# zertovitch/zip-ada

Hardware: AMD Instinct MI355X
Metric: Deflate encode MB/s (Deflate_3; stream bit-exact with the CPU restatement of the reference, Ada parity unpinned) (higher is better)
Workload: dtype u8

## Files before the change

### zip-ada_amd/csrc/zada_logic.h

```cpp
#pragma once
#include <type_traits>
#include <stdint.h>

#if defined(__HIPCC__)
#define ZADA_HD __host__ __device__ __forceinline__
#else
#define ZADA_HD inline
#endif

namespace zada {

constexpr uint32_t TOK_MATCH = 0x80000000u;
ZADA_HD uint32_t tok_match(uint32_t len, uint32_t dist) { return TOK_MATCH | (len << 16) | dist; }
ZADA_HD bool tok_is_match(uint32_t t) { return (t & TOK_MATCH) != 0; }
ZADA_HD uint32_t tok_len(uint32_t t) { return tok_is_match(t) ? ((t >> 16) & 0x1FF) : 1u; }
ZADA_HD uint32_t tok_dist(uint32_t t) { return t & 0xFFFF; }

constexpr int MIN_MATCH = 3, MAX_MATCH = 258, MAX_DIST = 32506, TOO_FAR = 4096;
constexpr int WSIZE = 32768;

struct LzConfig { int good, lazy, nice, chain; };
ZADA_HD LzConfig lz_config(int level) {
  switch (level) {
    case 4: return {4, 4, 16, 16};
// ... 71 lines not shown
}


struct MatchPair { uint32_t full, quarter; };
constexpr uint32_t M_GUESS = 0x80000000u, M_DEMAND = 0x40000000u, M_BYSPEC = 0x20000000u, M_HAVEQ = 0x10000000u, M_VALUE = 0x01FFFFFFu;
constexpr uint32_t M_BEAT_SHIFT = 25, M_BEAT_MAX = 127;
struct NoGuess { ZADA_HD void operator()(uint32_t, uint32_t, uint32_t, uint32_t) const {} };
struct ParseIO { const uint8_t *in; uint64_t n; const MatchPair *M; LzConfig cfg; const uint32_t *segend; };
struct Layout { const uint32_t *segend; uint64_t n; };
struct ExitState { uint32_t pos, kind; };

struct BitmapWriter {
  uint32_t *bits; uint64_t word; uint32_t acc;
  ZADA_HD void init(uint32_t *b, uint64_t first) { bits = b; acc = 0; word = first; }
  ZADA_HD void set(uint64_t p) {
    uint64_t w = p >> 5;
    while (word < w) { bits[word] = acc; acc = 0; word++; }
    acc |= 1u << (p & 31);
  }
  ZADA_HD void finish(uint64_t last) {
    while (word < last) { bits[word] = acc; acc = 0; word++; }
    bits[word] = acc;
  }
};

struct DirectFetch { const MatchPair *M; ZADA_HD MatchPair operator()(uint32_t p) const { return M[p]; } };
template <typename F> struct has_byte { template <typename U> static auto test(int) -> decltype(((U *)0)->byte(0u), char()); template <typename U> static long test(...); static const bool value = sizeof(test<F>(0)) == 1; };
template <typename F> ZADA_HD typename std::enable_if<has_byte<typename std::remove_reference<F>::type>::value, uint32_t>::type fetch_byte(F &f, const uint8_t *, uint32_t p) { return f.byte(p); }
template <typename F> ZADA_HD typename std::enable_if<!has_byte<typename std::remove_reference<F>::type>::value, uint32_t>::type fetch_byte(F &, const uint8_t *in, uint32_t p) { return in[p]; }
struct DirectSink { uint32_t *tok; uint32_t &ntok; ZADA_HD void push(uint32_t t) { tok[ntok++] = t; } };
struct CappedSink { uint32_t *tok; uint32_t &ntok; uint32_t cap; uint32_t *overflow; ZADA_HD void push(uint32_t t) { if (ntok < cap) tok[ntok] = t; else if (overflow) *overflow = 1u; ntok++; } };
template <typename Sink, typename OnTop, typename OnGuess, typename Fetch>
ZADA_HD void run_parser(ParseState &s, const ParseIO &io, Sink &&sink, OnTop &&on_top, OnGuess &&on_guess, Fetch &&fetch) {
  for (;;) {
    if ((uint64_t)s.p >= io.n) {
      if (s.avail) { sink.push(io.in[io.n - 1]); s.avail = 0; s.mlen = 2; }
      return;
    }
    if (on_top(s)) return;
    const uint64_t la = io.n - s.p;
    const bool srch = parse_searches(s, io.cfg, la);
    uint32_t m = 0;
    if (srch) {
      const MatchPair mm = fetch(s.p);
      if (mm.full & M_GUESS) on_guess(s.p, mm.full, mm.quarter, s.mlen);
      m = (parse_need_quarter(s, io.cfg) ? mm.quarter : mm.full) & M_VALUE;
    }
    const uint32_t bb = s.avail ? fetch_byte(fetch, io.in, s.p - 1) : 0;
    const uint32_t t = parse_step(s, m, srch, bb);
    if (t != 0xFFFFFFFFu) sink.push(t);
  }
}

template <typename Sink, typename OnGuess, typename Fetch>
ZADA_HD void parse_spec_chunk_to(const ParseIO &io, uint32_t k, uint32_t chunk, Sink &&sink,
                                 uint32_t *Fbits, uint32_t *Lbits, ExitState &ex, OnGuess on_guess, Fetch &&fetch) {
  const uint64_t c0 = (uint64_t)k * chunk, c1 = (c0 + chunk < io.n) ? c0 + chunk : io.n;
  ParseState s{(uint32_t)c0, 0, 2, 0};
  BitmapWriter fw, lw;
  fw.init(Fbits, c0 >> 5); lw.init(Lbits, c0 >> 5);
  ExitState e; e.pos = (uint32_t)io.n; e.kind = SYNC_F;
  run_parser(s, io, sink, [&](const ParseState &st) {
    int kind = sync_kind(st);
    if (kind == SYNC_NONE) return false;
    if ((uint64_t)st.p >= c1) { e.pos = st.p; e.kind = (uint32_t)kind; return true; }
    if (kind == SYNC_F) fw.set(st.p); else lw.set(st.p);
    return false;
  }, on_guess, fetch);
  const uint64_t lastw = c1 > c0 ? (c1 - 1) >> 5 : c0 >> 5;
  fw.finish(lastw);
  lw.finish(lastw);
  ex = e;
}
template <typename OnGuess, typename Fetch>
ZADA_HD void parse_spec_chunk(const ParseIO &io, uint32_t k, uint32_t chunk, uint32_t *tok, uint32_t &ntok,
                              uint32_t *Fbits, uint32_t *Lbits, ExitState &ex, OnGuess on_guess, Fetch &&fetch) {
  parse_spec_chunk_to(io, k, chunk, DirectSink{tok, ntok}, Fbits, Lbits, ex, on_guess, fetch);
}
ZADA_HD void parse_spec_chunk(const ParseIO &io, uint32_t k, uint32_t chunk, uint32_t *tok, uint32_t &ntok,
                              uint32_t *Fbits, uint32_t *Lbits, ExitState &ex) {
  parse_spec_chunk_to(io, k, chunk, DirectSink{tok, ntok}, Fbits, Lbits, ex, NoGuess(), DirectFetch{io.M});
}

template <typename OnGuess, typename Fetch>
ZADA_HD void parse_fix_chunk(const ParseIO &io, uint32_t k, uint32_t chunk, ExitState entry,
                             const uint32_t *spec_tok, uint32_t spec_cnt, const uint32_t *Fbits, const uint32_t *Lbits,
                             ExitState spec_exit, uint32_t *tok, uint32_t &ntok, uint32_t &take, uint32_t &u0, ExitState &new_exit,
                             OnGuess on_guess, Fetch &&fetch, uint32_t tok_cap = 0xFFFFFFFFu, uint32_t *tok_overflow = nullptr) {
  const uint64_t c0 = (uint64_t)k * chunk, c1 = (c0 + chunk < io.n) ? c0 + chunk : io.n;
  u0 = entry.kind == SYNC_L ? entry.pos - 1 : entry.pos;
  ntok = 0;
  if ((uint64_t)entry.pos >= c1) {
    new_exit = entry; take = spec_cnt;
    return;
  }
  ParseState s{entry.pos, entry.kind == SYNC_L ? 1u : 0u, 2, 0};
  bool synced = false;
  ExitState e; e.pos = (uint32_t)io.n; e.kind = SYNC_F;
  run_parser(s, io, CappedSink{tok, ntok, tok_cap, tok_overflow}, [&](const ParseState &st) {
    int kind = sync_kind(st);
    if (kind == SYNC_NONE) return false;
    if ((uint64_t)st.p >= c1) { e.pos = st.p; e.kind = (uint32_t)kind; return true; }
    uint32_t wbits = (kind == SYNC_F ? Fbits : Lbits)[st.p >> 5];
    if ((wbits >> (st.p & 31)) & 1) { synced = true; e.pos = st.p; e.kind = (uint32_t)kind; return true; }
    return false;
  }, on_guess, fetch);
  if (synced) {
    const uint32_t u = e.kind == SYNC_L ? e.pos - 1 : e.pos;
    uint32_t cur = (uint32_t)c0, j = 0;
    while (cur < u) { cur += tok_len(spec_tok[j]); j++; }
    take = j;
    new_exit = spec_exit;
  } else {
    take = spec_cnt;
    new_exit = e;
  }
}
ZADA_HD void parse_fix_chunk(const ParseIO &io, uint32_t k, uint32_t chunk, ExitState entry,
                                    const uint32_t *spec_tok, uint32_t spec_cnt, const uint32_t *Fbits, const uint32_t *Lbits,
                                    ExitState spec_exit, uint32_t *tok, uint32_t &ntok, uint32_t &take, uint32_t &u0, ExitState &new_exit) {
  parse_fix_chunk(io, k, chunk, entry, spec_tok, spec_cnt, Fbits, Lbits, spec_exit, tok, ntok, take, u0, new_exit, NoGuess(), DirectFetch{io.M});
}

template <typename T>
ZADA_HD void patch_dist_stats(T *sd) {
  int used = 0;
  for (int i = 0; i < 32; i++) if (sd[i] != 0) used++;
  if (used == 0) { sd[0] = 1; sd[1] = 1; }
  else if (used == 1) { if (sd[0] == 0) sd[0] = 1; else sd[1] = 1; }
}

ZADA_HD void tweak_for_better_rle(uint32_t *counts, int counts_len, uint8_t *good) {
  int length = counts_len, stride;
  uint32_t symbol, sum, limit, new_count;
  for (int i = 0; i < counts_len; i++) good[i] = 0;
  for (;;) { if (length == 0) return; if (counts[length - 1] != 0) break; length--; }
  symbol = counts[0]; stride = 0;
  for (int i = 0; i <= length; i++) {
    if (i == length || counts[i] != symbol) {
      if ((symbol == 0 && stride >= 5) || (symbol != 0 && stride >= 7))
        for (int k = 0; k < stride; k++) good[i - k - 1] = 1;
      stride = 1;
      if (i != length) symbol = counts[i];
    } else stride++;
  }
  stride = 0; limit = counts[0]; sum = 0;
  for (int i = 0; i <= length; i++) {
    bool brk = (i == length) || good[i] || (i > 0 && good[i - 1]);
    if (!brk) { int64_t d = (int64_t)counts[i] - (int64_t)limit; if (d < 0) d = -d; brk = d >= 4; }
    if (brk) {
      if (stride >= 4 || (stride >= 3 && sum == 0)) {
        new_count = (sum + (uint32_t)stride / 2) / (uint32_t)stride;
        if (new_count < 1) new_count = 1;
        if (sum == 0) new_count = 0;
        for (int k = 0; k < stride; k++) counts[i - k - 1] = new_count;
      }
      stride = 0; sum = 0;
      if (i < length - 3) limit = (counts[i] + counts[i + 1] + counts[i + 2] + counts[i + 3] + 2) / 4;
      else if (i < length) limit = counts[i];
      else limit = 0;
    }
    stride++;
    if (i != length) sum += counts[i];
  }
}

// ... 62 lines not shown
```

### zip-ada_amd/csrc/zada_lz.hip

```cpp
#include <hip/hip_runtime.h>
#include <mutex>
#include <stdint.h>
#include "zada_logic.h"
#include "zada_internal.h"
#include <chrono>
#include <stdio.h>
#include <stdlib.h>
#include <vector>

namespace zada {

typedef uint32_t __attribute__((aligned(1))) u32u;
typedef uint64_t __attribute__((aligned(1))) u64u;
#define RL(v, j) ((uint32_t)__builtin_amdgcn_readlane((int)(v), (j)))
#define RL64(v, j) ((uint64_t)RL((uint32_t)(v), (j)) | ((uint64_t)RL((uint32_t)((v) >> 32), (j)) << 32))

#ifndef ZADA_NO_XCD_MAP
__device__ __forceinline__ uint32_t xcd_block() {
  const uint32_t n = gridDim.x, full = n & ~7u, b = blockIdx.x;
  return b < full ? (b & 7u) * (full >> 3) + (b >> 3) : b;
}
#else
__device__ __forceinline__ uint32_t xcd_block() { return blockIdx.x; }
#endif
// ... 1373 lines not shown
      };
      uint32_t s_end = lds_u32(WI + (uint32_t)bst - 3);
      bool over = false;
      auto batch = [&](uint32_t d) {
        const bool valid = d != 0;
        const bool inr = valid && d <= LF;
        bool pass = false;
        if (inr) pass = lds_u32(WI - d + (uint32_t)bst - 3) == s_end;
        unsigned long long pm = __ballot(pass);
        while (pm) {
          const int j = __ffsll((long long)pm) - 1;
          const uint32_t dj = RL(d, j);
          if (!hq && dj > LQ) { hq = true; rqq = bst >= 3 ? ((uint32_t)bst << 16) | bd : 0u; }
          const uint32_t o = 4u * (uint32_t)lane;
          const uint32_t x = lds_u32(WI - dj + o) ^ lds_u32(WI + o);
          const unsigned long long mm = __ballot(x != 0);
          int len;
          if (mm) { const int l0 = __ffsll((long long)mm) - 1; len = 4 * l0 + (int)(__builtin_ctz(RL(x, l0)) >> 3); }
          else { const uint32_t y = LDS_U16(win8, WI - dj + 256) ^ LDS_U16(win8, WI + 256); len = 256 + (y == 0 ? 2 : ((y & 0xFF) == 0 ? 1 : 0)); }
          len = len < LA ? len : LA;
          if (len > bst) {
            bst = len; bd = dj;
            if (len >= NICE) { over = true; break; }
            s_end = lds_u32(WI + (uint32_t)bst - 3);
            pass = pass && lane > j && lds_u32(WI - d + (uint32_t)bst - 3) == s_end;
          } else pass = pass && lane > j;
          pm = __ballot(pass);
        }
        if (!over && !hq && __any(valid && d > LQ)) { hq = true; rqq = bst >= 3 ? ((uint32_t)bst << 16) | bd : 0u; }
        if (__any(!inr)) over = true;
      };
      uint32_t dq[DM_AHEAD];
      dq[0] = r0;
#pragma unroll
      for (int u = 1; u < DM_AHEAD; u++) dq[u] = 64u * u < TT ? cand_load(ds, 64u * u + (uint32_t)lane) : 0u;
      for (uint32_t c0 = 0; c0 < TT && !over; c0 += 64 * DM_AHEAD) {
#pragma unroll
        for (int u = 0; u < DM_AHEAD; u++) {
          if (c0 + 64u * u < TT && !over) {
            const uint32_t dcur = cand_dist(ds, c0 + 64u * u + (uint32_t)lane, dq[u]);
            const uint32_t cn = c0 + 64u * (u + DM_AHEAD);
            if (cn < TT) dq[u] = cand_load(ds, cn + (uint32_t)lane);
            batch(dcur);
          }
        }
      }
      if (lane == 0) {
        const uint32_t packed = bst >= 3 ? ((uint32_t)bst << 16) | bd : 0u;
        store_result(B + ds.k, packed, hq ? rqq : packed, ds.og_full, ds.og_quarter, (ds.best_hq >> 14) & 1u);
      }
    }
    __syncthreads();
    DM_STAMP(3);
  }
}

__global__ void k_demand_all(Layout L, MatchPair *__restrict__ M, uint32_t *__restrict__ blk_demand, uint32_t *__restrict__ dbits) {
  const uint64_t p = (uint64_t)blockIdx.x * blockDim.x + threadIdx.x;
  if (p >= L.n || p >= lay_end(L, p >> 15)) return;
  const uint32_t f = M[p].full;
  if (f & M_GUESS) {
    if (!(f & M_DEMAND)) M[p].full = f | M_DEMAND | M_BYSPEC;
    atomicOr(&dbits[p >> 5], 1u << (p & 31));
    blk_demand[p / DMB] = 1;
  }
}

struct DemandMarker {
  MatchPair *M; uint32_t *blk_demand; uint32_t *n_demand; uint32_t by;
  bool track = false;
  uint32_t *dbits;
  __device__ void operator()(uint32_t p, uint32_t full, uint32_t quarter, uint32_t beat) const {
    if (track && (beat < M_BEAT_MAX ? beat : M_BEAT_MAX) < (quarter >> M_BEAT_SHIFT))
      __hip_atomic_fetch_min(&M[p].quarter, (quarter & M_VALUE) | ((beat < M_BEAT_MAX ? beat : M_BEAT_MAX) << M_BEAT_SHIFT), __ATOMIC_RELAXED, __HIP_MEMORY_SCOPE_AGENT);
    const uint32_t want = M_DEMAND | by;
    if ((full & want) == want) return;
    M[p].full = full | want;
    atomicOr(&dbits[p >> 5], 1u << (p & 31));
    blk_demand[p / DMB] = 1;
    *n_demand = 1;
  }
};

#ifndef ZADA_PS_BWORDS
#define ZADA_PS_BWORDS 16
#endif
#ifndef ZADA_PS_TOKS
#define ZADA_PS_TOKS 8
#endif
constexpr uint32_t PS_BWORDS = ZADA_PS_BWORDS, PS_TOKS = ZADA_PS_TOKS;
static_assert((PS_BWORDS == 8 || PS_BWORDS == 16) && (PS_TOKS == 4 || PS_TOKS == 8), "line sizes of the parser's LDS caches");
struct LineFetch {
  const MatchPair *M; uint64_t *slot;
  uint32_t tag;
  __device__ MatchPair operator()(uint32_t p) {
    const uint32_t t = p >> 3;
    if (t != tag) {
      const uint4 *src = (const uint4 *)(M + ((uint64_t)t << 3));
      const uint4 a = src[0], b = src[1], c = src[2], d = src[3];
      slot[0 * 64] = (uint64_t)a.x | ((uint64_t)a.y << 32); slot[1 * 64] = (uint64_t)a.z | ((uint64_t)a.w << 32);
      slot[2 * 64] = (uint64_t)b.x | ((uint64_t)b.y << 32); slot[3 * 64] = (uint64_t)b.z | ((uint64_t)b.w << 32);
      slot[4 * 64] = (uint64_t)c.x | ((uint64_t)c.y << 32); slot[5 * 64] = (uint64_t)c.z | ((uint64_t)c.w << 32);
      slot[6 * 64] = (uint64_t)d.x | ((uint64_t)d.y << 32); slot[7 * 64] = (uint64_t)d.z | ((uint64_t)d.w << 32);
      tag = t;
    }
    const uint64_t v = slot[(p & 7u) * 64];
    MatchPair r; r.full = (uint32_t)v; r.quarter = (uint32_t)(v >> 32);
    return r;
  }
  const uint8_t *in; uint32_t *bslot; uint32_t btag;
  __device__ uint32_t byte(uint32_t p) {
    constexpr uint32_t SH = PS_BWORDS == 16 ? 6 : 5;
    const uint32_t t = p >> SH;
    if (t != btag) {
      const uint4 *src = (const uint4 *)(in + ((uint64_t)t << SH));
      const uint4 a = src[0], b = src[1];
      bslot[0 * 64] = a.x; bslot[1 * 64] = a.y; bslot[2 * 64] = a.z; bslot[3 * 64] = a.w;
      bslot[4 * 64] = b.x; bslot[5 * 64] = b.y; bslot[6 * 64] = b.z; bslot[7 * 64] = b.w;
      if (PS_BWORDS == 16) {
        const uint4 c = src[2], d = src[3];
        bslot[8 * 64] = c.x; bslot[9 * 64] = c.y; bslot[10 * 64] = c.z; bslot[11 * 64] = c.w;
        bslot[12 * 64] = d.x; bslot[13 * 64] = d.y; bslot[14 * 64] = d.z; bslot[15 * 64] = d.w;
      }
      btag = t;
    }
    return (bslot[((p >> 2) & (PS_BWORDS - 1u)) * 64] >> (8 * (p & 3u))) & 0xFFu;
  }
};

struct TokSink {
  uint32_t *dst; uint32_t *buf; uint32_t n;
  __device__ void push(uint32_t t) {
    buf[(n & (PS_TOKS - 1u)) * 64] = t;
    n++;
    if ((n & (PS_TOKS - 1u)) == 0) {
      uint4 a;
      a.x = buf[0]; a.y = buf[64]; a.z = buf[128]; a.w = buf[192];
      uint4 *o = (uint4 *)(dst + n - PS_TOKS);
      o[0] = a;
      if (PS_TOKS == 8) { uint4 b; b.x = buf[256]; b.y = buf[320]; b.z = buf[384]; b.w = buf[448]; o[1] = b; }
    }
  }
  __device__ void flush() { for (uint32_t i = n & ~(PS_TOKS - 1u); i < n; i++) dst[i] = buf[(i & (PS_TOKS - 1u)) * 64]; }
};

__global__ void __launch_bounds__(1024) k_list_flagged(const uint8_t *__restrict__ flag, uint32_t n, uint32_t *__restrict__ list, uint32_t *__restrict__ count) {
  __shared__ uint32_t wcnt[16], wbase;
  const uint32_t i = blockIdx.x * 1024 + threadIdx.x, lane = threadIdx.x & 63, w = threadIdx.x >> 6;
  const bool f = i < n && flag[i];
  const unsigned long long mk = __ballot(f);
  if (lane == 0) wcnt[w] = (uint32_t)__popcll(mk);
  __syncthreads();
  if (threadIdx.x == 0) {
    uint32_t t = 0;
    for (int k = 0; k < 16; k++) { const uint32_t c = wcnt[k]; wcnt[k] = t; t += c; }
    wbase = t ? atomicAdd(count, t) : 0u;
  }
  __syncthreads();
  if (f) list[wbase + wcnt[w] + (uint32_t)__popcll(mk & ((1ull << lane) - 1ull))] = i;
}

#ifdef ZADA_RESPEC_STATS
__device__ unsigned long long g_respec_dbg[4];
#endif
__global__ void k_parse_spec(ParseIO io, uint32_t nchunks, uint32_t *__restrict__ spec_tok, uint32_t *__restrict__ spec_cnt,
                             uint32_t *__restrict__ Fbits, uint32_t *__restrict__ Lbits, ExitState *__restrict__ exits,
                             DemandMarker dm, const uint32_t *__restrict__ list , const uint32_t *__restrict__ list_n,
                             uint32_t exact_max ) {
  uint32_t k = blockIdx.x * blockDim.x + threadIdx.x;
  if (list) {
    const uint32_t nl = *list_n;
    if (nl <= exact_max || k >= nl) return;
    k = list[k];
  }
  if (k >= nchunks) return;
  if (io.segend) io.n = io.segend[((uint64_t)k * PCHUNK) >> 15] & 0x7FFFFFFFu;
  uint32_t ntok = 0;
  ExitState ex;
#ifdef ZADA_RESPEC_STATS
  uint32_t old_h = 0, old_n = 0; ExitState old_ex{0, 0};
  if (list) { old_n = spec_cnt[k]; old_ex = exits[k]; const uint32_t *ot = spec_tok + (uint64_t)k * PTOK_STRIDE; for (uint32_t i = 0; i < old_n; i++) old_h = old_h * 0x9E3779B1u + ot[i]; }
#endif
  __shared__ uint64_t lines[8 * 64];
  __shared__ uint32_t tbuf[PS_TOKS * 64];
  __shared__ uint32_t blines[PS_BWORDS * 64];
  LineFetch lf; lf.M = io.M; lf.slot = lines + threadIdx.x; lf.tag = 0xFFFFFFFFu; lf.in = io.in; lf.bslot = blines + threadIdx.x; lf.btag = 0xFFFFFFFFu;
  TokSink ts; ts.dst = spec_tok + (uint64_t)k * PTOK_STRIDE; ts.buf = tbuf + threadIdx.x; ts.n = 0;
  parse_spec_chunk_to(io, k, PCHUNK, ts, Fbits, Lbits, ex, dm, lf);
  ts.flush();
  ntok = ts.n;
  spec_cnt[k] = ntok;
  exits[k] = ex;
#ifdef ZADA_RESPEC_STATS
  if (list) {
    __threadfence();
    uint32_t new_h = 0; const uint32_t *nt = spec_tok + (uint64_t)k * PTOK_STRIDE; for (uint32_t i = 0; i < ntok; i++) new_h = new_h * 0x9E3779B1u + nt[i];
    atomicAdd(&g_respec_dbg[0], 1ull);
    if (new_h == old_h && ntok == old_n && ex.pos == old_ex.pos && ex.kind == old_ex.kind) atomicAdd(&g_respec_dbg[1], 1ull);
  }
#endif
}

struct WaveExact {
  const uint8_t *in; Layout L; DistPlanes dp; RunPtrs rp; const uint16_t *tailsK; MatchPair *M; int nice_cfg; const uint16_t *resume;
  __device__ __forceinline__ uint32_t g32(uint64_t o) const { return *(const u32u *)(in + o); }
  __device__ MatchPair search(uint64_t p, MatchPair og) const {
    const int lane = threadIdx.x & 63;
    const uint64_t seg = p >> 15, n = lay_end(L, seg);
    const bool seg_first = lay_first(L, seg), prev_first = seg > 0 && lay_first(L, seg - 1);
    const uint64_t rem = n - p;
    const int la = rem < 258 ? (int)rem : 258;
    const int nice = nice_cfg < la ? nice_cfg : la;
    const uint64_t pbase = (seg << 15) - 32768;
    const uint32_t dlimv = dp.limits(p);
    uint32_t dl[NLEVELS];
#pragma unroll
    for (int l = 0; l < NLEVELS; l++) dl[l] = dp.d[l][p];
    const uint32_t idx1 = rp.idx[p], c1 = rp.cnt[p];
    uint32_t t = 0xFFFFu;
    if (!seg_first) {
      const uint32_t key = hashL_of(*(const u64u *)(in + p), 3 + NLEVELS);
      const uint32_t tt = tailsK[(seg - 1) * 65536ull + key];
      const uint64_t q = pbase + tt;
      if (tt < lay_inserted(L, seg - 1) && p - q <= (uint64_t)MAX_DIST && hashL_of(*(const u64u *)(in + q), 3 + NLEVELS) == key) t = tt;
    }
    uint32_t idx2 = 0, c2 = 0;
    if (t != 0xFFFFu) { idx2 = rp.idx[pbase + t]; c2 = (uint32_t)rp.cnt[pbase + t] + 1u; }
    const uint32_t df = dlimv & 0xFFFF, dq = dlimv >> 16;
    const uint32_t LF = dl[0] == (uint32_t)MAX_DIST ? (uint32_t)MAX_DIST : (df < (uint32_t)(MAX_DIST - 1) ? df : (uint32_t)(MAX_DIST - 1));
    const uint32_t LQ = dq < LF ? dq : LF;
    int bst = 2;
    uint32_t bd = 0, rqq = 0;
    bool chain_ok = true;
#pragma unroll
    for (int l = 0; l < NLEVELS; l++) {
      const bool v = la >= 3 + l && dl[l] != 0 && dl[l] <= LF;
      if (v) { bst = 3 + l; bd = dl[l]; if (dl[l] <= LQ) rqq = ((uint32_t)(3 + l) << 16) | dl[l]; }
      chain_ok = v;
    }
    bool hq = chain_ok && bd > LQ;
    uint32_t i1 = idx1, n1 = c1, i2 = idx2, n2 = c2;
    if (chain_ok) {
      const uint32_t gl = (og.full & M_VALUE) >> 16;
      if (gl >= 3) { bst = (int)gl; bd = og.full & 0xFFFFu; }
      hq = (og.full & M_HAVEQ) != 0;
      if (hq) rqq = og.quarter & M_VALUE;
      const uint64_t q = p - resume[p];
      const uint32_t iq = rp.idx[q];
      const uint32_t skip = q >= (seg << 15) ? idx1 - 1 - iq : c1 + (idx2 - iq);
      if (skip < c1) { i1 = idx1 - skip; n1 = c1 - skip; }
      else { const uint32_t s2 = skip - c1 < c2 ? skip - c1 : c2; n1 = 0; i2 = idx2 - s2; n2 = c2 - s2; }
    }
    MatchPair r;
    if (!(chain_ok && bst < nice && n1 + n2 > 0)) {
      const uint32_t packed = bst >= 3 ? ((uint32_t)bst << 16) | bd : 0u;
      r.full = packed; r.quarter = !chain_ok ? rqq : (hq ? rqq : packed);
      if (lane == 0) M[p] = r;
      return r;
    }
    const uint16_t *sprev = rp.S + ((seg << 15) - 32768);
    const uint32_t TT = n1 + n2, po = (uint32_t)p & 32767u;
    auto cand = [&](uint32_t c) -> uint32_t {
      const bool in1 = c < n1, in2 = !in1 && c - n1 < n2;
      const uint32_t a = in1 ? 32768u + i1 - 1u - c : (in2 ? i2 - (c - n1) : 32768u);
      const uint32_t raw = sprev[a];
      const bool q0 = raw == 0 && ((in1 && seg_first) || (in2 && prev_first));
      return q0 ? 0u : (in1 ? po - raw : (in2 ? po + 32768u - raw : 0u));
    };
    uint32_t s_end = g32(p + (uint32_t)bst - 3);
    bool over = false;
    uint32_t dnext = cand((uint32_t)lane);
    for (uint32_t c0 = 0; c0 < TT && !over; c0 += 64) {
      const uint32_t d = dnext;
      if (c0 + 64 < TT) dnext = cand(c0 + 64 + (uint32_t)lane);
      const bool valid = d != 0;
      const bool inr = valid && d <= LF;
      bool pass = false;
      if (inr) pass = g32(p - d + (uint32_t)bst - 3) == s_end;
      unsigned long long pm = __ballot(pass);
      while (pm) {
        const int j = __ffsll((long long)pm) - 1;
        const uint32_t dj = RL(d, j);
// ... 341 lines not shown
        const uint32_t s1 = s0 + PIECE < nseg ? s0 + PIECE : nseg;
        const uint64_t upto = (uint64_t)s1 * 32768 + 64 < n ? (uint64_t)s1 * 32768 + 64 : n;
        if (int rn = job.need(upto)) return rn;
        const auto t_now = std::chrono::steady_clock::now();
        const bool slow = s0 > 0 && std::chrono::duration<double>(t_now - t_prev).count() >= SLOW_PIECE_S;
        t_prev = t_now;
        prev_links(s0, s1);
#ifndef ZADA_OLD_INIT
        if (s0 == 0) hipStreamWaitEvent(st, c->ev_dlim, 0);
#endif
        if (slow) cross_links_upto(s1);
        hipLaunchKernelGGL(k_bucket_limits, dim3(s1 - s0), dim3(256), 0, st, L, cfg.chain, cfg.chain >> 2, W.S3, W.bsc3, W.dlim, W.dlim_bits, W.segmax, W.heavy, s0);
        s0 = s1;
      }
      if (int rn = job.need(n)) return rn;
      cross_links_upto(nseg);
      if (nseg > 1) cross_dist();
    } else
    prev_links(0, nseg);
#ifndef ZADA_OLD_INIT
    if (!job.need) hipStreamWaitEvent(st, c->ev_dlim, 0);
#endif
#ifdef ZADA_PL_STATS
    { unsigned long long h[32]; hipMemcpy(h, W.dbg, sizeof h, hipMemcpyDeviceToHost); fprintf(stderr, "[prev_links cycles/segment] init %.0f |", (double)h[8] / nseg); for (int q = 9; q < 9 + 4 * (NLEVELS + 1) - 1; q++) fprintf(stderr, " %.0f", (double)h[q] / nseg); fprintf(stderr, "  (per level 3..: sort, links, first candidates, queue rounds)\n"); fprintf(stderr, "[level 4 walks per segment] rounds %.2f  entries %.1f  entries of the last round %.1f  hops there %.1f (max %llu over all segments; walks over 64 hops %.3f)  first-queue overflow %.1f  cycles of the last round %.0f\n", (double)h[24] / nseg, (double)h[25] / nseg, (double)h[26] / nseg, (double)h[27] / nseg, h[28], (double)h[29] / nseg, (double)h[30] / nseg, (double)h[31] / nseg); hipMemset(W.dbg, 0, 256);
      unsigned long long sd[8]; hipMemcpyFromSymbol(sd, HIP_SYMBOL(g_sort_dbg), sizeof sd); fprintf(stderr, "[sort_pass cycles/segment, all six passes] clear %.0f  rank (LDS atomics) %.0f  scan %.0f  scatter %.0f\n", (double)sd[0] / nseg, (double)sd[1] / nseg, (double)sd[2] / nseg, (double)sd[3] / nseg); for (int q = 0; q < 8; q++) sd[q] = 0; hipMemcpyToSymbol(HIP_SYMBOL(g_sort_dbg), sd, sizeof sd); }
#endif
    c->tmark("prev_links");
    if (!job.need) {
      if (nseg > 1) {
        cross_links(1, nseg);
        cross_dist();
      }
      hipLaunchKernelGGL(k_bucket_limits, dim3(nseg), dim3(256), 0, st, L, cfg.chain, cfg.chain >> 2, W.S3, W.bsc3, W.dlim, W.dlim_bits, W.segmax, W.heavy, 0u);
    }
  }
#ifdef ZADA_CD_STATS
  { unsigned long long h[16]; hipDeviceSynchronize(); hipMemcpyFromSymbol(h, HIP_SYMBOL(g_cd_dbg), sizeof h);
    fprintf(stderr, "[k_cross_dist level-4 walks] %llu walks (%.1f %% of the positions), %llu steps (%.2f per walk), found %llu (%.1f %%), no step %llu, > 8 steps %llu, > 64 steps %llu, steps of the walks that found nothing %llu, gave-up restarts %llu\n",
            h[0], 100.0 * h[0] / n, h[1], (double)h[1] / (h[0] ? h[0] : 1), h[2], 100.0 * h[2] / (h[0] ? h[0] : 1), h[3], h[4], h[5], h[6], h[7]);
    fprintf(stderr, "[k_cross_dist level-4 walks] > 32 steps %llu, > 128 %llu, > 256 %llu, > 512 %llu, > 1024 %llu, longest %llu\n", h[8], h[9], h[10], h[11], h[12], h[13]);
    for (int q = 0; q < 16; q++) h[q] = 0; hipMemcpyToSymbol(HIP_SYMBOL(g_cd_dbg), h, sizeof h); }
#endif
  c->tmark("cross_links");
  const uint32_t nbm = (uint32_t)((n + MB - 1) / MB);
  const uint32_t nch = (uint32_t)((n + PCHUNK - 1) / PCHUNK);
  const int max_rounds = c->knob_max_demand_rounds;
  int budget_env = c->knob_budget >= 0 ? c->knob_budget : (n < (2u << 20) ? 0 : n < (512u << 20) ? 8 : 6);
  if (budget_env < 1) budget_env = 1 << 20;
  const uint32_t nbd = (uint32_t)((n + DMB - 1) / DMB);
  hipMemsetAsync(W.blk_demand, 0, (size_t)nbd * 4, st);
  hipMemsetAsync(W.dbits, 0, (size_t)nbd * (DMB / 8), st);
  hipMemsetAsync(W.n_demand, 0, 4, st);
  hipLaunchKernelGGL(k_match, dim3(nbm), dim3(1024), MATCH_LDS, st, W.in, L, W.lprev[NLEVELS - 1], dpl, W.M, cfg.nice,
                     budget_env, (unsigned long long *)W.dbg, W.lprev[0], budget_env > c->knob_inner_budget ? c->knob_inner_budget : 0);
  c->tmark("match");
  ParseIO io; io.in = W.in; io.n = n; io.M = W.M; io.cfg = cfg; io.segend = job.segend;
  DemandMarker dm; dm.M = W.M; dm.blk_demand = W.blk_demand; dm.n_demand = W.n_demand; dm.by = M_BYSPEC; dm.dbits = W.dbits;
  DemandMarker dmf = dm; dmf.by = 0;
  int rounds = 0, demand_rounds = 0;
  bool valve_used = false;
  static const bool round_stats = getenv("ZADA_ROUND_STATS") != nullptr;
  const ExitState entry0 = job.entry_known ? job.entry : ExitState{0, SYNC_F};
  const uint32_t kE = job.entry_known ? (entry0.pos / PCHUNK < nch ? entry0.pos / PCHUNK : nch) : 0u;
  hipMemsetAsync(W.n_changed + 6, 0, 4, st);
  bool restart = false, first_again = false;
  for (bool first = true;; first = false) {
    if (first_again) { first = true; first_again = false; }
    const bool beat_valid = !first;
    if (first) hipLaunchKernelGGL(k_parse_spec, dim3((nch + 63) / 64), dim3(64), 0, st, io, nch,
                                  W.spec_tok, W.spec_cnt, W.Fbits, W.Lbits, W.spec_exits, dm, (const uint32_t *)nullptr, (const uint32_t *)nullptr, 0u);
    else {
      hipMemsetAsync(W.n_changed + 2, 0, 4, st);
      hipLaunchKernelGGL(k_list_flagged, dim3((nch + 1023) / 1024), dim3(1024), 0, st, W.chg, nch, W.offsets, W.n_changed + 2);
      const uint32_t exact_max = c->knob_exact_respec > 0 ? (uint32_t)c->knob_exact_respec : 0u;
      if (exact_max) {
        WaveExact wx; wx.in = W.in; wx.L = L; wx.dp = dpl; wx.rp = rpt; wx.tailsK = W.ltails[NLEVELS - 1]; wx.M = W.M; wx.nice_cfg = cfg.nice; wx.resume = W.lprev[0];
        hipLaunchKernelGGL(k_parse_spec_exact, dim3(256 * 5), dim3(64 * PX_WAVES), 0, st, io, nch, W.spec_tok, W.spec_cnt, W.Fbits, W.Lbits, W.spec_exits,
                           wx, (const uint32_t *)W.offsets, (const uint32_t *)(W.n_changed + 2), exact_max);
      }
      DemandMarker dmt = dm; dmt.track = true;
      hipLaunchKernelGGL(k_parse_spec, dim3((nch + 63) / 64), dim3(64), 0, st, io, nch,
                         W.spec_tok, W.spec_cnt, W.Fbits, W.Lbits, W.spec_exits, dmt, (const uint32_t *)W.offsets, (const uint32_t *)(W.n_changed + 2), exact_max);
    }
    hipMemcpyAsync(W.true_exits, W.spec_exits, (size_t)nch * sizeof(ExitState), hipMemcpyDeviceToDevice, st);
    if (kE > 0) hipLaunchKernelGGL(k_seed_entry, dim3((kE + 255) / 256), dim3(256), 0, st, W.true_exits, kE, entry0);
    hipMemsetAsync(W.dirty[0], 1, nch, st);
    int cur = 0, it = 0;
    uint32_t ndem = 0;
    bool slow = false;
    for (;;) {
      hipMemsetAsync(W.dirty[cur ^ 1], 0, nch, st);
      hipMemsetAsync(W.n_changed, 0, 4, st);
      hipMemsetAsync(W.n_changed + 1, 0xFF, 4, st);
      hipLaunchKernelGGL(k_parse_fix, dim3((nch + 63) / 64), dim3(64), 0, st, io, nch,
                         W.spec_tok, W.spec_cnt, W.Fbits, W.Lbits, W.spec_exits, W.true_exits, W.fix_tok, W.fix_cnt,
                         W.take_from, W.start_pos, W.dirty[cur], W.dirty[cur ^ 1], W.n_changed, dmf, entry0, W.fix_stride, W.n_changed + 6);
      hipLaunchKernelGGL(k_fix_forward, dim3(1), dim3(64), 0, st, io, nch, W.true_exits, W.dirty[cur ^ 1], W.n_changed);
      uint32_t changed = 0, fix_ovf = 0;
      hipMemcpyAsync(&changed, W.n_changed, 4, hipMemcpyDeviceToHost, st);
      hipMemcpyAsync(&ndem, W.n_demand, 4, hipMemcpyDeviceToHost, st);
      if (W.fix_stride < PTOK_STRIDE) hipMemcpyAsync(&fix_ovf, W.n_changed + 6, 4, hipMemcpyDeviceToHost, st);
      if (hip_check(c, hipStreamSynchronize(st), "parse_fix")) return ZADA_E_HIP_;
      rounds++;
      if (fix_ovf) {
        uint32_t *bigger = nullptr;
        const uint64_t nch_cap = W.cap_n / PCHUNK + 2;
        if (hipMalloc(&bigger, nch_cap * (uint64_t)PTOK_STRIDE * 4) != hipSuccess) { (void)hipGetLastError(); c->err = "out of device memory (splice tokens)"; return -2; }
        W.allocs.push_back(bigger);
        W.fix_tok = bigger; W.fix_stride = PTOK_STRIDE;
        c->fix_grown++;
        hipMemsetAsync(W.n_changed + 6, 0, 4, st);
        restart = true;
        break;
      }
      if (changed == 0) break;
      if (++it >= 32 && !valve_used) { slow = true; break; }
      cur ^= 1;
    }
    if (round_stats) {
      uint32_t nl = 0, nmark = 0;
      if (!first) hipMemcpy(&nl, W.n_changed + 2, 4, hipMemcpyDeviceToHost);
      { std::vector<uint32_t> hb(nbd); hipMemcpy(hb.data(), W.blk_demand, (size_t)nbd * 4, hipMemcpyDeviceToHost); for (uint32_t v : hb) nmark += v != 0; }
      fprintf(stderr, "[lz round %d] %s parse of %u chunks, splice iterations so far %d, blocks with demanded positions %u of %u, demand %u%s\n", demand_rounds, first || nl > (uint32_t)(c->knob_exact_respec > 0 ? c->knob_exact_respec : 0) ? "speculative" : "exact",
              first ? nch : nl, rounds, nmark, nbd, ndem, slow ? " (slow splice)" : "");
    }
#ifdef ZADA_RESPEC_STATS
    if (!first) { unsigned long long h[4]; hipDeviceSynchronize(); hipMemcpyFromSymbol(h, HIP_SYMBOL(g_respec_dbg), sizeof h); fprintf(stderr, "[respec round %d] %llu chunks parsed again, %llu of them with the same tokens and exit as before\n", demand_rounds, h[0], h[1]); h[0] = h[1] = 0; hipMemcpyToSymbol(HIP_SYMBOL(g_respec_dbg), h, sizeof h); }
#endif
    if (restart) { restart = false; first_again = true; continue; }
    if (ndem == 0 && !slow) break;
    demand_rounds++;
    if (demand_rounds > 1000) { c->err = "demand loop did not converge"; return ZADA_E_HIP_; }
    hipMemsetAsync(W.n_demand, 0, 4, st);
    hipMemsetAsync(W.chg, 0, nch, st);
    if ((demand_rounds == max_rounds || slow) && !valve_used) {
      valve_used = true;
      hipLaunchKernelGGL(k_demand_all, dim3((uint32_t)((n + 255) / 256)), dim3(256), 0, st, L, W.M, W.blk_demand, W.dbits);
    }
    hipLaunchKernelGGL(k_match_demand, dim3(nbd), dim3(DM_THREADS), DM_LDS, st, W.in, L, dpl, rpt, W.ltails[NLEVELS - 1], W.M, cfg.nice,
                       W.blk_demand, W.dbits, W.chg, W.spec_exits, W.lprev[0], beat_valid);
    hipMemsetAsync(W.blk_demand, 0, (size_t)nbd * 4, st);
#ifdef ZADA_DM_STATS
    { unsigned long long h[8]; hipDeviceSynchronize(); hipMemcpyFromSymbol(h, HIP_SYMBOL(g_dm_dbg), sizeof h);
      fprintf(stderr, "[k_match_demand round %d] %llu blocks, %.1f marked positions and %.1f scans per block; cycles per block: staging %.0f, list %.0f, phase A %.0f, phase B %.0f\n", demand_rounds, h[4],
              (double)h[5] / (h[4] ? h[4] : 1), (double)h[6] / (h[4] ? h[4] : 1), (double)h[0] / (h[4] ? h[4] : 1), (double)h[1] / (h[4] ? h[4] : 1), (double)h[2] / (h[4] ? h[4] : 1), (double)h[3] / (h[4] ? h[4] : 1));
      for (int q = 0; q < 8; q++) h[q] = 0; hipMemcpyToSymbol(HIP_SYMBOL(g_dm_dbg), h, sizeof h); }
#endif
  }
  c->demand_rounds += demand_rounds;
  c->parse_rounds += rounds;
  c->tmark("parse");
  const uint32_t k0 = job.tok_lo / PCHUNK, k1 = job.final ? nch : job.tok_hi / PCHUNK, nk = k1 - k0;
  if (nk == 0) { c->err = "empty shard"; return -1; }
  hipLaunchKernelGGL(k_tok_count, dim3((nch + 255) / 256), dim3(256), 0, st, nch, W.spec_cnt, W.fix_cnt, W.take_from, W.counts);
  exclusive_scan_u32(st, W.counts + k0, W.offsets, W.scan_sums, W.n_changed, nk);
  struct { uint32_t total; ExitState ex, warm; } h;
  h.ex = ExitState{(uint32_t)n, SYNC_F}; h.warm = ExitState{0, SYNC_F};
  hipMemcpyAsync(&h.total, W.n_changed, 4, hipMemcpyDeviceToHost, st);
  if (!job.final) hipMemcpyAsync(&h.ex, W.true_exits + (k1 - 1), sizeof(ExitState), hipMemcpyDeviceToHost, st);
  if (k0 > 0) hipMemcpyAsync(&h.warm, W.true_exits + (k0 - 1), sizeof(ExitState), hipMemcpyDeviceToHost, st);
  if (hip_check(c, hipStreamSynchronize(st), "tok_scan")) return ZADA_E_HIP_;
  uint32_t *dst_atoms = job.dst_atoms, *dst_apos = job.dst_apos;
  if (h.total > job.cap_atoms) {
    if (!job.grow_atoms) { c->err = "atom array overflow"; return -2; }
    if (int rg = job.grow_atoms(h.total, &dst_atoms, &dst_apos)) return rg;
  }
// ... 9 lines not shown
```

Measured before the change: 9454.

## Stage parser inputs per phase into LDS instead of lazy per-line fetch

Replaces the lazy tag-checked line caches in the speculative parse kernel with a phased loop. Each wave stages a fixed window of match pairs and input bytes into LDS for every lane in bulk, parses up to the phase end, then repeats until every lane finishes its chunk. The goal is to batch and overlap the global loads across lanes rather than stalling on divergent per-lane cache misses. The cost is extra wave-wide iterations while lanes diverge, and redundant staging when a phase's window is only partly consumed. Optional stats instrumentation is added behind a macro.

```diff
diff --git a/zip-ada_amd/csrc/zada_logic.h b/zip-ada_amd/csrc/zada_logic.h
--- a/zip-ada_amd/csrc/zada_logic.h
+++ b/zip-ada_amd/csrc/zada_logic.h
@@ -177,6 +177,46 @@
   parse_spec_chunk_to(io, k, chunk, DirectSink{tok, ntok}, Fbits, Lbits, ex, NoGuess(), DirectFetch{io.M});
 }
 
+struct PhasedParse {
+  ParseState s; BitmapWriter fw, lw; uint64_t c0, c1;
+#ifdef ZADA_PS_STATS
+  uint32_t turns;
+#endif
+};
+enum { PHASE_PAUSE = 0, PHASE_EXIT = 1 };
+ZADA_HD void parse_phased_begin(PhasedParse &ps, const ParseIO &io, uint32_t k, uint32_t chunk, uint32_t *Fbits, uint32_t *Lbits) {
+  ps.c0 = (uint64_t)k * chunk; ps.c1 = (ps.c0 + chunk < io.n) ? ps.c0 + chunk : io.n;
+  ps.s = ParseState{(uint32_t)ps.c0, 0, 2, 0};
+  ps.fw.init(Fbits, ps.c0 >> 5); ps.lw.init(Lbits, ps.c0 >> 5);
+#ifdef ZADA_PS_STATS
+  ps.turns = 0;
+#endif
+}
+ZADA_HD uint32_t parse_phase_start(const PhasedParse &ps, uint32_t Q) { return ps.s.p & ~(Q - 1u); }
+template <typename Sink, typename OnGuess, typename Fetch>
+ZADA_HD int parse_spec_chunk_phased(PhasedParse &ps, const ParseIO &io, uint32_t Q, Sink &&sink, ExitState &ex, OnGuess on_guess, Fetch &&fetch) {
+  const uint64_t phase_end = (uint64_t)parse_phase_start(ps, Q) + Q, c1 = ps.c1;
+  BitmapWriter &fw = ps.fw, &lw = ps.lw;
+  bool paused = false;
+  ExitState e; e.pos = (uint32_t)io.n; e.kind = SYNC_F;
+  run_parser(ps.s, io, sink, [&](const ParseState &st) {
+    const int kind = sync_kind(st);
+    if (kind != SYNC_NONE && (uint64_t)st.p >= c1) { e.pos = st.p; e.kind = (uint32_t)kind; return true; }
+    if ((uint64_t)st.p >= phase_end) { paused = true; return true; }
+#ifdef ZADA_PS_STATS
+    ps.turns++;
+#endif
+    if (kind == SYNC_F) fw.set(st.p); else if (kind == SYNC_L) lw.set(st.p);
+    return false;
+  }, on_guess, fetch);
+  if (paused) return PHASE_PAUSE;
+  const uint64_t lastw = c1 > ps.c0 ? (c1 - 1) >> 5 : ps.c0 >> 5;
+  fw.finish(lastw);
+  lw.finish(lastw);
+  ex = e;
+  return PHASE_EXIT;
+}
+
 template <typename OnGuess, typename Fetch>
 ZADA_HD void parse_fix_chunk(const ParseIO &io, uint32_t k, uint32_t chunk, ExitState entry,
                              const uint32_t *spec_tok, uint32_t spec_cnt, const uint32_t *Fbits, const uint32_t *Lbits,
diff --git a/zip-ada_amd/csrc/zada_lz.hip b/zip-ada_amd/csrc/zada_lz.hip
--- a/zip-ada_amd/csrc/zada_lz.hip
+++ b/zip-ada_amd/csrc/zada_lz.hip
@@ -1479,51 +1479,51 @@
   }
 };
 
-#ifndef ZADA_PS_BWORDS
-#define ZADA_PS_BWORDS 16
+#ifndef ZADA_PS_PHASE
+#define ZADA_PS_PHASE 16
 #endif
 #ifndef ZADA_PS_TOKS
 #define ZADA_PS_TOKS 8
 #endif
-constexpr uint32_t PS_BWORDS = ZADA_PS_BWORDS, PS_TOKS = ZADA_PS_TOKS;
-static_assert((PS_BWORDS == 8 || PS_BWORDS == 16) && (PS_TOKS == 4 || PS_TOKS == 8), "line sizes of the parser's LDS caches");
-struct LineFetch {
-  const MatchPair *M; uint64_t *slot;
-  uint32_t tag;
-  __device__ MatchPair operator()(uint32_t p) {
-    const uint32_t t = p >> 3;
-    if (t != tag) {
-      const uint4 *src = (const uint4 *)(M + ((uint64_t)t << 3));
-      const uint4 a = src[0], b = src[1], c = src[2], d = src[3];
-      slot[0 * 64] = (uint64_t)a.x | ((uint64_t)a.y << 32); slot[1 * 64] = (uint64_t)a.z | ((uint64_t)a.w << 32);
-      slot[2 * 64] = (uint64_t)b.x | ((uint64_t)b.y << 32); slot[3 * 64] = (uint64_t)b.z | ((uint64_t)b.w << 32);
-      slot[4 * 64] = (uint64_t)c.x | ((uint64_t)c.y << 32); slot[5 * 64] = (uint64_t)c.z | ((uint64_t)c.w << 32);
-      slot[6 * 64] = (uint64_t)d.x | ((uint64_t)d.y << 32); slot[7 * 64] = (uint64_t)d.z | ((uint64_t)d.w << 32);
-      tag = t;
-    }
-    const uint64_t v = slot[(p & 7u) * 64];
+constexpr uint32_t PS_Q = ZADA_PS_PHASE, PS_TOKS = ZADA_PS_TOKS;
+constexpr uint32_t PS_BW = PS_Q / 4 + 1;
+static_assert((PS_Q == 8 || PS_Q == 16 || PS_Q == 32 || PS_Q == 64) && PCHUNK % PS_Q == 0 && (PS_TOKS == 4 || PS_TOKS == 8), "phase and token buffer of the parser's LDS");
+struct PhaseFetch {
+  const uint64_t *slot; const uint32_t *bslot;
+  uint32_t start;
+  __device__ MatchPair operator()(uint32_t p) const {
+    const uint64_t v = slot[(p - start) * 64];
     MatchPair r; r.full = (uint32_t)v; r.quarter = (uint32_t)(v >> 32);
     return r;
   }
-  const uint8_t *in; uint32_t *bslot; uint32_t btag;
-  __device__ uint32_t byte(uint32_t p) {
-    constexpr uint32_t SH = PS_BWORDS == 16 ? 6 : 5;
-    const uint32_t t = p >> SH;
-    if (t != btag) {
-      const uint4 *src = (const uint4 *)(in + ((uint64_t)t << SH));
-      const uint4 a = src[0], b = src[1];
-      bslot[0 * 64] = a.x; bslot[1 * 64] = a.y; bslot[2 * 64] = a.z; bslot[3 * 64] = a.w;
-      bslot[4 * 64] = b.x; bslot[5 * 64] = b.y; bslot[6 * 64] = b.z; bslot[7 * 64] = b.w;
-      if (PS_BWORDS == 16) {
-        const uint4 c = src[2], d = src[3];
-        bslot[8 * 64] = c.x; bslot[9 * 64] = c.y; bslot[10 * 64] = c.z; bslot[11 * 64] = c.w;
-        bslot[12 * 64] = d.x; bslot[13 * 64] = d.y; bslot[14 * 64] = d.z; bslot[15 * 64] = d.w;
-      }
-      btag = t;
-    }
-    return (bslot[((p >> 2) & (PS_BWORDS - 1u)) * 64] >> (8 * (p & 3u))) & 0xFFu;
+  __device__ uint32_t byte(uint32_t p) const {
+    const uint32_t o = p + 4u - start;
+    return (bslot[(o >> 2) * 64] >> (8 * (o & 3u))) & 0xFFu;
   }
 };
+__device__ __forceinline__ void ps_stage(bool live, uint32_t start, uint64_t n, const MatchPair *__restrict__ M, const uint8_t *__restrict__ in,
+                                         uint64_t *slot, uint32_t *bslot) {
+  if (!live || (uint64_t)start >= n) return;
+  uint4 r[PS_Q / 2]; uint2 b[PS_Q / 8];
+#pragma unroll
+  for (uint32_t j = 0; j < PS_Q / 8; j++) {
+    const uint64_t at = (uint64_t)start + 8 * j < n ? (uint64_t)start + 8 * j : (uint64_t)start;
+    const uint4 *src = (const uint4 *)(M + at);
+    r[4 * j] = src[0]; r[4 * j + 1] = src[1]; r[4 * j + 2] = src[2]; r[4 * j + 3] = src[3];
+    b[j] = *(const uint2 *)(in + at);
+  }
+  const uint32_t b0 = *(const uint32_t *)(in + (start > 0 ? (uint64_t)start - 4 : 0));
+  bslot[0] = b0;
+#pragma unroll
+  for (uint32_t j = 0; j < PS_Q / 8; j++) {
+#pragma unroll
+    for (uint32_t q = 0; q < 4; q++) {
+      const uint4 v = r[4 * j + q];
+      slot[(8 * j + 2 * q) * 64] = (uint64_t)v.x | ((uint64_t)v.y << 32); slot[(8 * j + 2 * q + 1) * 64] = (uint64_t)v.z | ((uint64_t)v.w << 32);
+    }
+    bslot[(1 + 2 * j) * 64] = b[j].x; bslot[(2 + 2 * j) * 64] = b[j].y;
+  }
+}
 
 struct TokSink {
   uint32_t *dst; uint32_t *buf; uint32_t n;
@@ -1560,41 +1560,82 @@
 #ifdef ZADA_RESPEC_STATS
 __device__ unsigned long long g_respec_dbg[4];
 #endif
-__global__ void k_parse_spec(ParseIO io, uint32_t nchunks, uint32_t *__restrict__ spec_tok, uint32_t *__restrict__ spec_cnt,
+#ifdef ZADA_PS_STATS
+__device__ unsigned long long g_ps_dbg[8];
+__device__ __forceinline__ uint32_t ps_wave_max(uint32_t v) { for (int o = 32; o > 0; o >>= 1) { const uint32_t w = (uint32_t)__shfl_xor((int)v, o); v = w > v ? w : v; } return v; }
+__device__ __forceinline__ uint32_t ps_wave_sum(uint32_t v) { for (int o = 32; o > 0; o >>= 1) v += (uint32_t)__shfl_xor((int)v, o); return v; }
+#endif
+__global__ void __launch_bounds__(64) k_parse_spec(ParseIO io, uint32_t nchunks, uint32_t *__restrict__ spec_tok, uint32_t *__restrict__ spec_cnt,
                              uint32_t *__restrict__ Fbits, uint32_t *__restrict__ Lbits, ExitState *__restrict__ exits,
                              DemandMarker dm, const uint32_t *__restrict__ list , const uint32_t *__restrict__ list_n,
                              uint32_t exact_max ) {
   uint32_t k = blockIdx.x * blockDim.x + threadIdx.x;
+  bool live = true;
   if (list) {
     const uint32_t nl = *list_n;
-    if (nl <= exact_max || k >= nl) return;
-    k = list[k];
-  }
-  if (k >= nchunks) return;
-  if (io.segend) io.n = io.segend[((uint64_t)k * PCHUNK) >> 15] & 0x7FFFFFFFu;
-  uint32_t ntok = 0;
+    if (nl <= exact_max) return;
+    live = k < nl;
+    if (live) k = list[k];
+  }
+  live = live && k < nchunks;
+  if (live && io.segend) io.n = io.segend[((uint64_t)k * PCHUNK) >> 15] & 0x7FFFFFFFu;
   ExitState ex;
 #ifdef ZADA_RESPEC_STATS
   uint32_t old_h = 0, old_n = 0; ExitState old_ex{0, 0};
-  if (list) { old_n = spec_cnt[k]; old_ex = exits[k]; const uint32_t *ot = spec_tok + (uint64_t)k * PTOK_STRIDE; for (uint32_t i = 0; i < old_n; i++) old_h = old_h * 0x9E3779B1u + ot[i]; }
-#endif
-  __shared__ uint64_t lines[8 * 64];
+  if (list && live) { old_n = spec_cnt[k]; old_ex = exits[k]; const uint32_t *ot = spec_tok + (uint64_t)k * PTOK_STRIDE; for (uint32_t i = 0; i < old_n; i++) old_h = old_h * 0x9E3779B1u + ot[i]; }
+#endif
+  __shared__ uint64_t lines[PS_Q * 64];
   __shared__ uint32_t tbuf[PS_TOKS * 64];
-  __shared__ uint32_t blines[PS_BWORDS * 64];
-  LineFetch lf; lf.M = io.M; lf.slot = lines + threadIdx.x; lf.tag = 0xFFFFFFFFu; lf.in = io.in; lf.bslot = blines + threadIdx.x; lf.btag = 0xFFFFFFFFu;
+  __shared__ uint32_t blines[PS_BW * 64];
   TokSink ts; ts.dst = spec_tok + (uint64_t)k * PTOK_STRIDE; ts.buf = tbuf + threadIdx.x; ts.n = 0;
-  parse_spec_chunk_to(io, k, PCHUNK, ts, Fbits, Lbits, ex, dm, lf);
-  ts.flush();
-  ntok = ts.n;
-  spec_cnt[k] = ntok;
-  exits[k] = ex;
+  PhasedParse ps;
+  if (live) parse_phased_begin(ps, io, k, PCHUNK, Fbits, Lbits);
+#ifdef ZADA_PS_STATS
+  if (!live) ps.turns = 0;
+  const unsigned long long ps_t0 = clock64();
+  unsigned long long ps_wait = 0, ps_loop = 0;
+  uint32_t ps_turns = 0, ps_events = 0, ps_lphases = 0;
+#endif
+  while (__ballot(live)) {
+#ifdef ZADA_PS_STATS
+    const unsigned long long ta = clock64();
+    const bool was_live = live;
+    const uint32_t turns0 = ps.turns;
+#endif
+    const uint32_t start = live ? parse_phase_start(ps, PS_Q) : 0u;
+    ps_stage(live, start, io.n, io.M, io.in, lines + threadIdx.x, blines + threadIdx.x);
+#ifdef ZADA_PS_STATS
+    asm volatile("s_waitcnt vmcnt(0) lgkmcnt(0)" ::: "memory");
+    const unsigned long long tb = clock64();
+    ps_lphases += live ? 1u : 0u;
+#endif
+    if (live) {
+      const PhaseFetch pf{lines + threadIdx.x, blines + threadIdx.x, start};
+      if (parse_spec_chunk_phased(ps, io, PS_Q, ts, ex, dm, pf) == PHASE_EXIT) {
+        live = false;
+        ts.flush();
+        spec_cnt[k] = ts.n;
+        exits[k] = ex;
 #ifdef ZADA_RESPEC_STATS
-  if (list) {
-    __threadfence();
-    uint32_t new_h = 0; const uint32_t *nt = spec_tok + (uint64_t)k * PTOK_STRIDE; for (uint32_t i = 0; i < ntok; i++) new_h = new_h * 0x9E3779B1u + nt[i];
-    atomicAdd(&g_respec_dbg[0], 1ull);
-    if (new_h == old_h && ntok == old_n && ex.pos == old_ex.pos && ex.kind == old_ex.kind) atomicAdd(&g_respec_dbg[1], 1ull);
-  }
+        if (list) {
+          __threadfence();
+          uint32_t new_h = 0; const uint32_t *nt = spec_tok + (uint64_t)k * PTOK_STRIDE; for (uint32_t i = 0; i < ts.n; i++) new_h = new_h * 0x9E3779B1u + nt[i];
+          atomicAdd(&g_respec_dbg[0], 1ull);
+          if (new_h == old_h && ts.n == old_n && ex.pos == old_ex.pos && ex.kind == old_ex.kind) atomicAdd(&g_respec_dbg[1], 1ull);
+        }
+#endif
+      }
+    }
+#ifdef ZADA_PS_STATS
+    const unsigned long long tc = clock64();
+    ps_wait += tb - ta; ps_loop += tc - tb; ps_events++;
+    ps_turns += ps_wave_max(was_live ? ps.turns - turns0 : 0u);
+#endif
+  }
+#ifdef ZADA_PS_STATS
+  { const uint32_t lt = ps_wave_sum(ps.turns), lp = ps_wave_sum(ps_lphases);
+    if (threadIdx.x == 0 && ps_events) { atomicAdd(&g_ps_dbg[0], 1ull); atomicAdd(&g_ps_dbg[1], (unsigned long long)ps_turns); atomicAdd(&g_ps_dbg[2], (unsigned long long)ps_events); atomicAdd(&g_ps_dbg[3], ps_wait);
+                            atomicAdd(&g_ps_dbg[4], ps_loop); atomicAdd(&g_ps_dbg[5], clock64() - ps_t0); atomicAdd(&g_ps_dbg[6], (unsigned long long)lt); atomicAdd(&g_ps_dbg[7], (unsigned long long)lp); } }
 #endif
 }
 
@@ -2102,6 +2143,12 @@
       hipLaunchKernelGGL(k_parse_spec, dim3((nch + 63) / 64), dim3(64), 0, st, io, nch,
                          W.spec_tok, W.spec_cnt, W.Fbits, W.Lbits, W.spec_exits, dmt, (const uint32_t *)W.offsets, (const uint32_t *)(W.n_changed + 2), exact_max);
     }
+#ifdef ZADA_PS_STATS
+    { unsigned long long h[8]; hipDeviceSynchronize(); hipMemcpyFromSymbol(h, HIP_SYMBOL(g_ps_dbg), sizeof h); const double w = h[0] ? (double)h[0] : 1.0;
+      fprintf(stderr, "[k_parse_spec round %d, Q %u] %llu waves; per wave: %.1f turns in %.1f phases, cycles %.0f = staging waits %.0f + loop %.0f; per lane with a chunk: %.1f turns in %.1f phases\n", demand_rounds, PS_Q, h[0],
+              (double)h[1] / w, (double)h[2] / w, (double)h[5] / w, (double)h[3] / w, (double)h[4] / w, (double)h[6] / (first ? (double)nch : w * 64.0), (double)h[7] / (first ? (double)nch : w * 64.0));
+      for (int q = 0; q < 8; q++) h[q] = 0; hipMemcpyToSymbol(HIP_SYMBOL(g_ps_dbg), h, sizeof h); }
+#endif
     hipMemcpyAsync(W.true_exits, W.spec_exits, (size_t)nch * sizeof(ExitState), hipMemcpyDeviceToDevice, st);
     if (kE > 0) hipLaunchKernelGGL(k_seed_entry, dim3((kE + 255) / 256), dim3(256), 0, st, W.true_exits, kE, entry0);
     hipMemsetAsync(W.dirty[0], 1, nch, st);
```

Measured after the change: 9408. About the same (-0.5%).
